# chsl/PLADE

Hardware: AMD Instinct MI355X
Metric: scan-pair registrations/sec, 1M-pt synthetic pairs (higher is better)
Workload: dtype f32

## Files before the change

### include/plade_hip.h

```cpp
#ifndef PLADE_HIP_H
#define PLADE_HIP_H
#include <stddef.h>
#include <stdint.h>
#ifdef __cplusplus
extern "C" {
#endif

#define PLADE_OK 0
#define PLADE_EINVAL (-1)
#define PLADE_EDEVICE (-2)
#define PLADE_ECAP (-3)
#define PLADE_EFAIL (-4)
#define PLADE_ELIMIT (-5)

#define PLADE_GROUP_MAX 8

typedef struct plade_ctx plade_ctx;
typedef struct plade_cloud plade_cloud;
typedef struct plade_comm plade_comm;

int plade_ctx_create(int device, plade_ctx **out);
void plade_ctx_destroy(plade_ctx *ctx);
const char *plade_last_error(const plade_ctx *ctx);
const char *plade_version(void);
// ... 382 lines not shown

int plade_dump_get(plade_ctx *ctx, const char *name, const void **ptr, int64_t *nbytes);
int plade_stats_get(plade_ctx *ctx, const char **names, const double **values, int32_t *count);
int plade_sort_pairs(plade_ctx *ctx, const void *keys, const uint32_t *vals, uint32_t n, int key_bytes, int bits,
                     void *keys_out, uint32_t *vals_out);
int plade_sort_segments(plade_ctx *ctx, const uint32_t *keys, const uint32_t *vals, const uint32_t *seg_off, uint32_t nseg, int bits,
                        uint32_t *keys_out, uint32_t *vals_out);

int plade_selftest_readback(plade_ctx *ctx, uint32_t n_ranges, uint32_t words, uint32_t *mismatches);

int plade_diag_launches(plade_ctx *ctx, uint32_t count, uint32_t blocks, uint32_t mbytes);
int plade_ply_read(const char *path, float **pos_nrm, uint64_t *n, char *err, size_t err_cap);
int plade_ply_read_points(const char *path, float **pos_nrm, uint64_t *n, int32_t *has_normals, char *err, size_t err_cap);
void plade_ply_free(float *pos_nrm);
int plade_diag_cluster_order(const float *sizes, uint32_t n, int32_t mode, int32_t depth_limit, int32_t *order);
int plade_diag_line_solver_host(int32_t kind, const float *a, const float *b, const float *c, const float *d, uint32_t n,
                                float *o1, float *o2, int32_t *ok);
int plade_kernel_time(plade_ctx *ctx, const char *which, int iters, double *avg_seconds,
                      double *algorithmic_bytes_per_launch);

#ifdef __cplusplus
}
#endif
#endif
```

### plade_amd/__init__.py

```python
import ctypes as C
import os
import numpy as np

_HERE = os.path.dirname(os.path.abspath(__file__))
LIB_PATH = os.path.join(_HERE, "libplade_hip.so")

PLADE_OK = 0
PLADE_EINVAL, PLADE_EDEVICE, PLADE_ECAP, PLADE_EFAIL, PLADE_ELIMIT = -1, -2, -3, -4, -5

ABI_SYMBOLS = [
    "plade_ctx_create", "plade_ctx_destroy", "plade_last_error", "plade_version", "plade_default_params",
    "plade_set_params", "plade_score_planes", "plade_extract_planes", "plade_match_descriptors",
    "plade_overlap_counts", "plade_average_spacing", "plade_voxel_downsample", "plade_registration_planes",
    "plade_registration", "plade_registration_minsupport", "plade_cloud_upload", "plade_cloud_free",
    "plade_registration_dev", "plade_dump_get", "plade_stats_get", "plade_kernel_time", "plade_plane_component",
    "plade_sort_pairs", "plade_host_pin", "plade_host_unpin", "plade_score_planes_subset", "plade_registration_next", "plade_cluster_transforms", "plade_device_synchronize", "plade_selftest_readback",
    "plade_registration_pairs", "plade_registration_pairs_dev", "plade_pair_ctx", "plade_set_candidate_shard", "plade_diag_launches", "plade_diag_cluster_order", "plade_diag_line_solver_host", "plade_sort_segments",
    "plade_closest_points", "plade_lines_meet", "plade_ply_read", "plade_ply_free",
    "plade_device_count", "plade_comm_unique_id", "plade_comm_create", "plade_comm_all_gather", "plade_comm_destroy", "plade_comm_last_error",
    "plade_set_candidate_shard_comm",
    "plade_estimate_normals", "plade_cloud_upload_xyz", "plade_ply_read_points",
    "plade_icp_default_params", "plade_refine_icp", "plade_refine_icp_dev", "plade_icp_linearize",
    "plade_cloud_distances", "plade_cloud_distances_dev",
    "plade_outlier_default_params", "plade_filter_outliers", "plade_cloud_filter_outliers_dev",
    "plade_merge_clouds", "plade_merge_clouds_dev", "plade_cloud_download",
    "plade_component_default_params", "plade_label_components", "plade_cloud_filter_components_dev",
    "plade_smooth_default_params", "plade_smooth_cloud", "plade_cloud_smooth_dev",
    "plade_gicp_default_params", "plade_refine_gicp", "plade_refine_gicp_dev", "plade_gicp_linearize",
    "plade_m3c2_default_params", "plade_cloud_m3c2", "plade_cloud_m3c2_dev",
    "plade_fpfh_default_params", "plade_cloud_fpfh", "plade_cloud_fpfh_dev", "plade_features_free",
    "plade_feature_match_default_params", "plade_match_features", "plade_match_features_dev",
    "plade_corr_pose_default_params", "plade_estimate_pose_corr", "plade_estimate_pose_corr_dev", "plade_corr_pose_moments",
# ... 176 lines not shown
    sig("plade_penetration_filter", argtypes=[p, p, u32, p, p, p, p, p, u32, p, p, p, p, p, u32, f, f, p, p, u64, p])
    sig("plade_overlap_counts", argtypes=[p, p, u32, p, u32, p, u32, p, f, f, p])
    sig("plade_average_spacing", argtypes=[p, p, u32, u32, u32, u32, p])
    sig("plade_voxel_downsample", argtypes=[p, p, u32, u32, f, p, p])
    sig("plade_registration_planes", argtypes=[p, p, u32, p, u32, p, p, p, u32, p, p, p, u32, p])
    sig("plade_registration", argtypes=[p, p, u32, p, u32, p])
    sig("plade_registration_next", argtypes=[p, p, u32, p, u32, p, u32, p, u32, p])
    sig("plade_registration_pairs", argtypes=[p, u32, p, p, p, p, u32, p, p, p, p, p, p])
    sig("plade_registration_pairs_dev", argtypes=[p, u32, p, p, p, p])
    sig("plade_pair_ctx", argtypes=[p, u32], restype=p)
    sig("plade_closest_points", argtypes=[p, i32, p, p, p, p, u32, p, p, p, p])
    sig("plade_lines_meet", argtypes=[p, i32, p, p, p, p, u32, p, p])
    sig("plade_diag_launches", argtypes=[p, u32, u32, u32])
    sig("plade_diag_cluster_order", argtypes=[p, u32, i32, i32, p])
    sig("plade_diag_line_solver_host", argtypes=[i32, p, p, p, p, u32, p, p, p])
    sig("plade_ply_read", argtypes=[C.c_char_p, C.POINTER(C.POINTER(C.c_float)), C.POINTER(u64), C.c_char_p, C.c_size_t])
    sig("plade_ply_free", argtypes=[C.POINTER(C.c_float)], restype=None)
    sig("plade_ply_read_points", argtypes=[C.c_char_p, C.POINTER(C.POINTER(C.c_float)), C.POINTER(u64), C.POINTER(i32), C.c_char_p,
                                           C.c_size_t])
    sig("plade_estimate_normals", argtypes=[p, p, u32, u32, i32, p, p, p, p])
    sig("plade_cloud_upload_xyz", argtypes=[p, p, u32, u32, i32, p, C.POINTER(p)])
    sig("plade_icp_default_params", argtypes=[C.POINTER(IcpParams)], restype=None)
    sig("plade_refine_icp", argtypes=[p, p, u32, p, u32, p, C.POINTER(IcpParams), p, C.POINTER(IcpResult)])
    sig("plade_refine_icp_dev", argtypes=[p, p, p, p, C.POINTER(IcpParams), p, C.POINTER(IcpResult)])
    sig("plade_icp_linearize", argtypes=[p, p, u32, p, u32, u32, p, p, f, p, p])
    sig("plade_gicp_default_params", argtypes=[C.POINTER(GicpParams)], restype=None)
    sig("plade_refine_gicp", argtypes=[p, p, u32, p, u32, p, C.POINTER(GicpParams), p, C.POINTER(GicpResult)])
    sig("plade_refine_gicp_dev", argtypes=[p, p, p, p, C.POINTER(GicpParams), p, C.POINTER(GicpResult)])
    sig("plade_gicp_linearize", argtypes=[p, p, u32, p, u32, p, p, f, C.c_double, p, p])
    sig("plade_cloud_distances", argtypes=[p, p, u32, p, u32, u32, p, f, p, p, p, C.POINTER(DistanceSummary)])
# ... 381 lines not shown
    if rc != 0:
        raise PladeError(rc, "plade_diag_line_solver_host failed")
    return (o1, o2, ok) if kind == 0 else (o1, ok)


def cluster_order(sizes, mode=0, depth_limit=-1):
    a = _f32(sizes).reshape(-1)
    out = np.zeros(len(a), np.int32)
    rc = load_library().plade_diag_cluster_order(a.ctypes.data_as(C.c_void_p), len(a), int(mode), int(depth_limit),
                                                 out.ctypes.data_as(C.c_void_p))
    if rc != 0:
        raise PladeError(rc, "plade_diag_cluster_order failed")
    return out


class Cloud:

    def __init__(self, ctx, pos_nrm, handle=None):
        self.ctx = ctx
        if handle is not None:
            self.n, self.h = handle
            return
        a = _f32(pos_nrm)
        if a.ndim != 2 or a.shape[1] != 6:
            raise ValueError(f"Cloud: an (N, 6) array x y z nx ny nz is required, got shape {a.shape}")
        self.n = len(a)
        self.h = C.c_void_p()
        ctx._check(ctx.L.plade_cloud_upload(ctx.h, _ptr(a), self.n, C.byref(self.h)))

    def download(self):
# ... 845 lines not shown
```

### plade_amd/csrc/combiner.hip

```cpp
#include "ctx.h"
#include <algorithm>

namespace plade {

namespace {
constexpr int RANGES_MAX = 32;
struct RangeArgs { const uint32_t *src[RANGES_MAX]; uint32_t *dst[RANGES_MAX]; uint32_t words[RANGES_MAX], value[RANGES_MAX], n; };

template <bool FILL>
__global__ __launch_bounds__(256) void k_ranges(const RangeArgs a, uint32_t *__restrict__ counter, uint32_t *flag, uint32_t seq) {
    const uint32_t r = blockIdx.y, n = a.words[r];
    uint32_t *__restrict__ dst = a.dst[r];
    if (FILL) {
        const uint32_t v = a.value[r];
        for (uint32_t i = blockIdx.x * 256u + threadIdx.x; i < n; i += gridDim.x * 256u) dst[i] = v;
    } else {
        const uint32_t *__restrict__ src = a.src[r];
        for (uint32_t i = blockIdx.x * 256u + threadIdx.x; i < n; i += gridDim.x * 256u) dst[i] = src[i];
    }
    if (!flag) return;
    __threadfence_system();
    __syncthreads();
    if (threadIdx.x == 0) {
        const uint32_t t = atomicAdd(counter, 1u);
// ... 28 lines not shown
    c->comb = this;
    c->comb_slot = slot;
    q[slot].clear();
    ++members;
    return slot;
}

QEntry &Combiner::push(plade_ctx *c) {
    std::vector<QEntry> &v = q[c->comb_slot];
    v.emplace_back();
    ++asked[c->comb_slot];
    return v.back();
}

static bool trace_lockstep() { static const bool v = getenv("PLADE_TRACE_LOCKSTEP") != nullptr; return v; }

void Combiner::flush_locked(std::unique_lock<std::mutex> &lk) {
    (void)lk;
    ++waits;
    const bool tr = trace_lockstep();
    const Clock::time_point t_in = Clock::now();
    size_t n_q = 0;
    uint64_t issued0 = launches_issued;
    if (tr) for (int s = 0; s < BATCH_MAX; ++s) n_q += q[s].size();
    Clock::time_point t_issued = t_in;
    struct TraceOut {
        Combiner *c; bool on; const Clock::time_point &t_in, &t_issued; size_t &n_q; uint64_t &issued0;
        ~TraceOut() {
            if (!on) return;
            const Clock::time_point t_out = Clock::now();
// ... 23 lines not shown
                if (n > best_n) { best_n = n; best = s; }
            }
            if (best < 0) break;
            const QEntry &lead_e = q[best][cur[best]];
            QEntry *es[BATCH_MAX];
            int n = 0;
            if (lead_e.kind == QEntry::FUNC) { es[n++] = &q[best][cur[best]]; ++cur[best]; }
            else
                for (int t = 0; t < BATCH_MAX; ++t) {
                    if (cur[t] >= q[t].size()) continue;
                    QEntry &f = q[t][cur[t]];
                    if (f.kind == lead_e.kind && f.id == lead_e.id) { es[n++] = &f; ++cur[t]; }
                }
            switch (es[0]->kind) {
                case QEntry::KERNEL:
                    es[0]->launch_many(st, n, es);
                    HIP_TRY(hipGetLastError());
                    ++launches_issued;
                    break;
                case QEntry::FUNC:
                    es[0]->fn(st);
                    HIP_TRY(hipGetLastError());
                    ++launches_issued;
                    break;
                case QEntry::COPY_IN:
                case QEntry::FILL: {
                    RangeArgs a;
                    memset(&a, 0, sizeof(a));
                    const QEntry::Kind kind = es[0]->kind;
                    auto put = [&](const QEntry &e) {
// ... 125 lines not shown
    c->read_arena_used = 0; c->write_arena_used = 0;
    c->comb = nullptr;
    c->comb_slot = -1;
}

void Combiner::bury(std::vector<void *> &gy) {
    std::lock_guard<std::mutex> lk(m);
    graveyard.insert(graveyard.end(), gy.begin(), gy.end());
    gy.clear();
}
Combiner::~Combiner() {
    for (void *p : graveyard) dev_free(p);
}

}
```

### plade_amd/csrc/k_overlap.hip

```cpp
#include "overlap.h"
#include "prims.h"

namespace plade {

struct GridParams {
    float mnx, mny, mnz, inv;
    int dx, dy, dz;
};

__device__ void k_minmax3(const VB &vb, const float *__restrict__ xyz, uint32_t n, uint32_t stride, float *__restrict__ out6) {
    __shared__ float s_lds[6][8];
    float mn[3] = {INFINITY, INFINITY, INFINITY}, mx[3] = {-INFINITY, -INFINITY, -INFINITY};
    for (uint32_t i = vb.bx * blockDim.x + threadIdx.x; i < n; i += vb.gx * blockDim.x)
        for (int k = 0; k < 3; ++k) {
            float v = xyz[(size_t)i * stride + k];
            mn[k] = fminf(mn[k], v);
            mx[k] = fmaxf(mx[k], v);
        }
    block_minmax_commit<3>(mn, mx, reinterpret_cast<int *>(out6), s_lds);
}

__device__ __forceinline__ uint32_t block_of(int cx, int cy, int cz, int dx, int dy) {
    const int bdx = (dx + 3) >> 2, bdy = (dy + 3) >> 2;
    return (uint32_t)((cx >> 2) + bdx * ((cy >> 2) + bdy * (cz >> 2)));
// ... 218 lines not shown
        return;
    }
    cell_start.ensure(ncells); cell_end.ensure(ncells);
    ctx->fill_async(cell_start.p, 0, ncells * 4);
    ctx->fill_async(cell_end.p, 0, ncells * 4);
    launch<k_gather_cells, 256>(ctx, dim3(cdiv(n, 256)), 0, d_xyz, stride, keys2.p, vals2.p, n,
                       sorted.p, cell_start.p, cell_end.p);
    HIP_TRY(hipGetLastError());
}

constexpr int OV_TPB = 256;
#ifndef OVD_W
#define OVD_W 5
#endif
constexpr int OV_KCH = 16;
constexpr uint32_t OV_MASK_MAX = 48u << 10;

__device__ void k_overlap(const VB &vb, const float *__restrict__ sx, const float *__restrict__ sy,
                                                    const float *__restrict__ sz, uint32_t n_s,
                                                    const float4 *__restrict__ tgt,
                                                    const unsigned long long *__restrict__ occ_bits,
                                                    const uint32_t *__restrict__ occ_rank,
                                                    const uint32_t *__restrict__ occ_start,
                                                    const float4 *__restrict__ cell_first,
                                                    const uint32_t *__restrict__ blk_mask, uint32_t mask_words, GridParams g,
                                                    const float *__restrict__ T ,
                                                    const float *__restrict__ centers , uint32_t K, float R2,
                                                    float r2, int32_t *__restrict__ counts, uint32_t ch, uint32_t items_per_wg) {
    __shared__ float s_T[OV_KCH][12];
    __shared__ float s_c[OV_KCH][3];
    __shared__ uint32_t s_cnt[OV_KCH];
    extern __shared__ uint32_t s_mask[];
    for (uint32_t i = threadIdx.x; i < mask_words; i += OV_TPB) s_mask[i] = blk_mask[i];
    const int lane = threadIdx.x & 63;
    const uint32_t ntiles = (n_s + OV_TPB - 1) / OV_TPB, nchunks = (K + ch - 1) / ch;
    const uint64_t nitems = (uint64_t)ntiles * nchunks;
    const uint64_t it0 = (uint64_t)vb.bx * items_per_wg, it1 = min(nitems, it0 + items_per_wg);
    uint32_t cur = 0xffffffffu, k0 = 0, kc = 0;
    for (uint64_t item = it0; item < it1; ++item) {
        const uint32_t chunk = (uint32_t)(item / ntiles), tile = (uint32_t)(item % ntiles);
        if (chunk != cur) {
            __syncthreads();
            if (cur != 0xffffffffu && threadIdx.x < kc && s_cnt[threadIdx.x]) atomicAdd(&counts[k0 + threadIdx.x], (int32_t)s_cnt[threadIdx.x]);
            __syncthreads();
            cur = chunk; k0 = chunk * ch; kc = min(ch, K - k0);
            for (uint32_t i = threadIdx.x; i < kc * 12; i += OV_TPB) s_T[i / 12][i % 12] = T[(size_t)(k0 + i / 12) * 16 + i % 12];
            for (uint32_t i = threadIdx.x; i < kc * 3; i += OV_TPB) s_c[i / 3][i % 3] = centers[(size_t)(k0 + i / 3) * 3 + i % 3];
            if (threadIdx.x < OV_KCH) s_cnt[threadIdx.x] = 0u;
            __syncthreads();
        }
        const uint32_t i = tile * OV_TPB + threadIdx.x;
        const bool live = i < n_s;
        const f3 p = live ? f3(sx[i], sy[i], sz[i]) : f3();
// ... 77 lines not shown
                }
            }
            const uint32_t h = (uint32_t)__popcll(__ballot(hit));
            if (lane == 0 && h) atomicAdd(&s_cnt[kk], h);
        }
    }
    __syncthreads();
    if (cur != 0xffffffffu && threadIdx.x < kc && s_cnt[threadIdx.x]) atomicAdd(&counts[k0 + threadIdx.x], (int32_t)s_cnt[threadIdx.x]);
}

__device__ void k_overlap_dense(const VB &vb, const float *__restrict__ sx, const float *__restrict__ sy, const float *__restrict__ sz,
                                uint32_t n_s, const float4 *__restrict__ tgt, const uint32_t *__restrict__ row_start,
                                const uint32_t *__restrict__ near_mask, uint32_t mask_words, int ms,
                                const uint32_t *__restrict__ row_occ , GridParams g,
                                const float *__restrict__ T , const float *__restrict__ centers , uint32_t K, float R2,
                                float r2, int32_t *__restrict__ counts, uint32_t ch, uint32_t items_per_wg) {
    __shared__ float s_T[OV_KCH][12];
    __shared__ float s_c[OV_KCH][3];
    __shared__ uint32_t s_cnt[OV_KCH];
    extern __shared__ uint32_t s_mask[];
    for (uint32_t i = threadIdx.x; i < mask_words; i += OV_TPB) s_mask[i] = near_mask[i];
    const int lane = threadIdx.x & 63;
    const uint32_t ntiles = (n_s + OV_TPB - 1) / OV_TPB, nchunks = (K + ch - 1) / ch;
    const uint64_t nitems = (uint64_t)ntiles * nchunks;
    const uint64_t it0 = (uint64_t)vb.bx * items_per_wg, it1 = min(nitems, it0 + items_per_wg);
    const uint32_t DX = (uint32_t)g.dx + 4u, DY = (uint32_t)g.dy + 4u;
    const uint32_t MBX = ((DX - 1u) >> ms) + 1u, MBY = ((DY - 1u) >> ms) + 1u;
    const uint32_t RS = DX, SS = DX * DY;
    const float fdx = (float)(g.dx + 1), fdy = (float)(g.dy + 1), fdz = (float)(g.dz + 1);
    uint32_t cur = 0xffffffffu, k0 = 0, kc = 0;
    for (uint64_t item = it0; item < it1; ++item) {
        const uint32_t chunk = (uint32_t)(item / ntiles), tile = (uint32_t)(item % ntiles);
        if (chunk != cur) {
            __syncthreads();
            if (cur != 0xffffffffu && threadIdx.x < kc && s_cnt[threadIdx.x]) atomicAdd(&counts[k0 + threadIdx.x], (int32_t)s_cnt[threadIdx.x]);
            __syncthreads();
            cur = chunk; k0 = chunk * ch; kc = min(ch, K - k0);
            for (uint32_t i = threadIdx.x; i < kc * 12; i += OV_TPB) s_T[i / 12][i % 12] = T[(size_t)(k0 + i / 12) * 16 + i % 12];
            for (uint32_t i = threadIdx.x; i < kc * 3; i += OV_TPB) s_c[i / 3][i % 3] = centers[(size_t)(k0 + i / 3) * 3 + i % 3];
            if (threadIdx.x < OV_KCH) s_cnt[threadIdx.x] = 0u;
            __syncthreads();
        }
        const uint32_t i = tile * OV_TPB + threadIdx.x;
        const bool live = i < n_s;
        const f3 p = live ? f3(sx[i], sy[i], sz[i]) : f3();
// ... 124 lines not shown
    if (!n_s) return;
    work.bbox.ensure(8);
    launch<k_init_minmax6, 64>(ctx, dim3(1), 0, work.bbox.p);
    launch<k_src_minmax, 256>(ctx, dim3(std::min(cdiv(n_s, 256), 512u)), 0, d_sx, d_sy, d_sz, n_s,
                       work.bbox.p);
    work.keys.ensure(n_s); work.keys2.ensure(n_s); work.vals.ensure(n_s); work.vals2.ensure(n_s);
    work.sorted.ensure(3 * (size_t)n_s + 4);
    launch<k_src_keys, 256>(ctx, dim3(cdiv(n_s, 256)), 0, d_sx, d_sy, d_sz, n_s, work.bbox.p, 1.f / cell,
                       work.keys.p, work.vals.p);
    sort_pairs_u32(ctx, work.keys.p, work.keys2.p, work.vals.p, work.vals2.p, n_s, 24);
    launch<k_src_gather, 256>(ctx, dim3(cdiv(n_s, 256)), 0, d_sx, d_sy, d_sz, n_s, work.vals2.p,
                       work.sorted.p);
    HIP_TRY(hipGetLastError());
}

void overlap_counts(plade_ctx *ctx, OverlapWork &work, const float *d_sx, const float *d_sy, const float *d_sz, uint32_t n_s,
                    const TargetGrid &grid, const float *d_T, const float *d_centers, uint32_t K, float src_radius,
                    float inlier_dist, int32_t *d_counts, uint32_t *d_any, bool counts_are_zero) {
    if (counts_are_zero) {}
    else if (reinterpret_cast<uint32_t *>(d_counts) + K == d_any) ctx->fill_async(d_counts, 0, (size_t)K * 8);
    else {
        ctx->fill_async(d_counts, 0, (size_t)K * 4);
        ctx->fill_async(d_any, 0, (size_t)K * 4);
    }
    if (K == 0 || grid.n == 0) return;
    const float R2 = pcl_r2((double)src_radius), r2 = pcl_r2((double)inlier_dist);
    GridParams g{grid.gp.mnx, grid.gp.mny, grid.gp.mnz, grid.gp.inv, grid.gp.dx, grid.gp.dy, grid.gp.dz};
    for (uint32_t k0 = 0; k0 < K; k0 += 2048) {
        uint32_t kc = std::min(2048u, K - k0);
        launch<k_sphere_any, 256>(ctx, dim3(cdiv(grid.n, 256)), kc * 12, grid.sorted.p, grid.n,
                           d_centers + (size_t)k0 * 3, kc, R2, d_any + k0);
    }
    if (n_s) {
        uint32_t ch = K <= 64 ? 2u : (K <= 512 ? 4u : (uint32_t)OV_KCH);
        if (grid.dense && K > 512) ch = 8u;
        const uint64_t nitems = (uint64_t)cdiv(n_s, OV_TPB) * cdiv(K, ch);
        const uint32_t fill = 256u * OVD_W / (uint32_t)std::max(1, ctx->comb ? ctx->comb->size() : 1);
        const uint32_t wgs = (uint32_t)std::min<uint64_t>(nitems, grid.dense ? std::max(64u, fill) : (ctx->comb ? 512u : 2048u));
        const uint32_t per = (uint32_t)((nitems + wgs - 1) / wgs);
        ctx->ev_begin("overlap", (double)K * n_s * 12.0 + (double)grid.n * 12.0);
        PLADE_REQUIRE(grid.compact, PLADE_EINVAL, "overlap: the target grid needs the compact occupancy index");
        if (grid.dense) {
            launch<k_overlap_dense, OV_TPB, OVD_W>(ctx, dim3(cdiv(nitems, per)), grid.mask_words * 4, d_sx, d_sy, d_sz, n_s, grid.sorted.p,
                               grid.row_start.p, grid.near_mask.p, grid.mask_words, grid.mask_shift,
                               grid.row_occ_on ? (const uint32_t *)grid.row_occ.p : (const uint32_t *)nullptr, g, d_T, d_centers, K, R2, r2, d_counts,
                               ch, per);
            ctx->ev_end();
            HIP_TRY(hipGetLastError());
            return;
        }
        const uint32_t nw = (uint32_t)((grid.ncells + 63) / 64);
        const uint32_t mask_words = (nw + 31) / 32 * 4 <= OV_MASK_MAX ? (nw + 63) / 64 * 2 : 0u;
        launch<k_overlap, OV_TPB, 5>(ctx, dim3(cdiv(nitems, per)), mask_words * 4, d_sx, d_sy, d_sz, n_s, grid.sorted.p,
                           grid.occ_bits.p, grid.occ_rank.p, grid.occ_start.p, grid.cell_first.p, reinterpret_cast<const uint32_t *>(grid.occ_blk.p), mask_words, g,
                           d_T, d_centers, K, R2, r2, d_counts, ch, per);
        ctx->ev_end();
    }
    HIP_TRY(hipGetLastError());
}

__global__ void k_deinterleave3(const float *__restrict__ xyz, uint32_t n, float *__restrict__ x, float *__restrict__ y,
                                float *__restrict__ z) {
    uint32_t i = blockIdx.x * blockDim.x + threadIdx.x;
    if (i >= n) return;
    x[i] = xyz[3 * (size_t)i]; y[i] = xyz[3 * (size_t)i + 1]; z[i] = xyz[3 * (size_t)i + 2];
}

void deinterleave3(plade_ctx *ctx, const float *d_xyz, uint32_t n, float *d_x, float *d_y, float *d_z) {
    if (!n) return;
    launch_raw(ctx, k_deinterleave3, dim3(cdiv(n, 256)), dim3(256), 0, d_xyz, n, d_x, d_y, d_z);
    HIP_TRY(hipGetLastError());
}

}

using namespace plade;

extern "C" int plade_overlap_counts(plade_ctx *ctx, const float *src_ds, uint32_t n_s, const float *tgt_ds,
                                    uint32_t n_t, const float *T, uint32_t k, const float *centers, float src_radius,
                                    float inlier_dist, int32_t *counts) {
    return guarded(ctx, [&]() -> int {
        PLADE_REQUIRE(src_ds && tgt_ds && T && centers && counts, PLADE_EINVAL, "plade_overlap_counts: null argument");
        DBuf<float> d_src, d_tgt, d_soa, d_T, d_c;
        DBuf<int32_t> d_counts;
        DBuf<uint32_t> d_any;
        d_src.ensure((size_t)n_s * 3 + 4); d_tgt.ensure((size_t)n_t * 3 + 4); d_soa.ensure((size_t)n_s * 3 + 4);
        d_T.ensure((size_t)k * 16 + 4); d_c.ensure((size_t)k * 3 + 4); d_counts.ensure(k + 1); d_any.ensure(k + 1);
        ctx->h2d(d_src.p, src_ds, (size_t)n_s * 12);
        ctx->h2d(d_tgt.p, tgt_ds, (size_t)n_t * 12);
        ctx->h2d(d_T.p, T, (size_t)k * 64);
        ctx->h2d(d_c.p, centers, (size_t)k * 12);
        deinterleave3(ctx, d_src.p, n_s, d_soa.p, d_soa.p + n_s, d_soa.p + 2 * (size_t)n_s);
        TargetGrid grid;
        grid.build(ctx, d_tgt.p, n_t, 3, inlier_dist, nullptr, nullptr, true);
        OverlapWork ow;
        if (n_t && n_s) overlap_sort_source(ctx, ow, d_soa.p, d_soa.p + n_s, d_soa.p + 2 * (size_t)n_s, n_s, 1.f / grid.gp.inv);
        else ow.sorted.ensure(3 * (size_t)n_s + 4);
        overlap_counts(ctx, ow, ow.sorted.p, ow.sorted.p + n_s, ow.sorted.p + 2 * (size_t)n_s, n_s, grid, d_T.p, d_c.p, k, src_radius,
                       inlier_dist, d_counts.p, d_any.p);
        std::vector<uint32_t> any(k);
        ctx->d2h(counts, d_counts.p, (size_t)k * 4);
        ctx->d2h(any.data(), d_any.p, (size_t)k * 4);
        ctx->sync();
        for (uint32_t i = 0; i < k; ++i)
            if (!any[i]) counts[i] = -1;
        return PLADE_OK;
    });
}
```

### plade_amd/csrc/launch.h

```cpp
#pragma once
#include "common.h"
#include <condition_variable>
#include <functional>
#include <mutex>
#include <type_traits>

struct plade_ctx;

namespace plade {

struct VB { uint32_t bx, by, gx, gy; };

constexpr int BATCH_MAX = 8;
constexpr size_t PACK_MAX = 464;

template <class... A> struct Pack;
template <> struct Pack<> {};
template <class H, class... T> struct Pack<H, T...> { H head; Pack<T...> tail; };

template <class... A> inline Pack<A...> make_pack(A... a);
template <> inline Pack<> make_pack<>() { return Pack<>{}; }
template <class H, class... T> inline Pack<H, T...> make_pack_impl(H h, T... t) { Pack<H, T...> p; p.head = h; p.tail = make_pack<T...>(t...); return p; }
template <class... A> inline Pack<A...> make_pack(A... a) { return make_pack_impl<A...>(a...); }

// ... 14 lines not shown

template <auto Body, int TPB, int N, class P, int MINW = 1>
__global__ __launch_bounds__(TPB, MINW) void k_batch(const BatchHdr h, const BatchPacks<P, N> packs) {
    uint32_t e = 0;
    if (N > 1) {
#pragma unroll
        for (int q = 1; q < N; ++q) e += (q < (int)h.n && blockIdx.x >= h.start[q]) ? 1u : 0u;
    }
    const uint32_t lin = blockIdx.x - h.start[e], gx = h.gx[e];
    VB vb;
    vb.bx = lin % gx; vb.by = lin / gx; vb.gx = gx; vb.gy = h.gy[e];
    call_body<Body>(vb, packs.p[e]);
}
#endif

struct QEntry {
    enum Kind : uint8_t { KERNEL, COPY_IN, FILL, FUNC } kind = KERNEL;
    const void *id = nullptr;
    void (*launch_many)(hipStream_t, int, QEntry *const *) = nullptr;
    uint32_t gx = 0, gy = 0, smem = 0;
    void *dst = nullptr; const void *src = nullptr; uint32_t words = 0, value = 0;
    std::function<void(hipStream_t)> fn;
    alignas(16) unsigned char pack[PACK_MAX];
};

struct Combiner {
    plade_ctx *lead = nullptr;
    std::mutex m;
    std::condition_variable cv;
    int members = 0, arrived = 0;
    uint64_t epoch = 0;
    std::string error;
    int error_code = 0;
    plade_ctx *member[BATCH_MAX] = {};
    std::vector<QEntry> q[BATCH_MAX];
// ... 31 lines not shown
        h.n = (uint32_t)k;
        for (int q = 0; q < k; ++q) {
            const QEntry &e = *es[b + q];
            h.gx[q] = std::max(1u, e.gx); h.gy[q] = std::max(1u, e.gy);
            h.start[q + 1] = h.start[q] + e.gx * e.gy;
            memcpy(static_cast<void *>(&packs.p[q]), e.pack, sizeof(P));
            smem = std::max(smem, e.smem);
        }
        for (int q = k; q < BATCH_MAX; ++q) h.start[q + 1] = h.start[k];
        if (h.start[k] == 0) continue;
        hipLaunchKernelGGL((k_batch<Body, TPB, N, P, MINW>), dim3(h.start[k]), dim3(TPB), smem, st, h, packs);
    }
}

template <auto Body, int TPB, int MINW = 1, class... Args>
void launch(plade_ctx *ctx, dim3 grid, size_t smem, Args... args) {
    using Tr = BodyTraits<decltype(Body)>;
    using P = typename Tr::pack;
    static_assert(std::is_trivially_copyable<P>::value, "kernel arguments must be plain data");
    const P p = Tr::make(args...);
    if (grid.x == 0 || grid.y == 0) return;
    Combiner *cb = ctx_combiner(ctx);
    if (!cb || sizeof(P) > PACK_MAX) {
        if (cb) {
            QEntry &e = cb->push(ctx);
            e.kind = QEntry::FUNC;
            e.fn = [p, grid, smem](hipStream_t st) {
                BatchHdr h; memset(&h, 0, sizeof(h));
                h.n = 1; h.gx[0] = grid.x; h.gy[0] = grid.y;
                for (int q = 0; q < BATCH_MAX; ++q) h.start[q + 1] = grid.x * grid.y;
                BatchPacks<P, 1> packs; packs.p[0] = p;
// ... 1 lines not shown
            };
            return;
        }
        BatchHdr h; memset(&h, 0, sizeof(h));
        h.n = 1; h.gx[0] = grid.x; h.gy[0] = grid.y;
        for (int q = 0; q < BATCH_MAX; ++q) h.start[q + 1] = grid.x * grid.y;
        BatchPacks<P, 1> packs; packs.p[0] = p;
        hipLaunchKernelGGL((k_batch<Body, TPB, 1, P, MINW>), dim3(grid.x * grid.y), dim3(TPB), smem, ctx_stream(ctx), h, packs);
        return;
    }
    QEntry &e = cb->push(ctx);
    e.kind = QEntry::KERNEL;
    e.launch_many = &launch_many_impl<Body, TPB, P, MINW>;
    e.id = reinterpret_cast<const void *>(e.launch_many);
    e.gx = grid.x; e.gy = grid.y; e.smem = (uint32_t)smem;
    memcpy(e.pack, static_cast<const void *>(&p), sizeof(P));
}
#endif

}
```

### plade_amd/csrc/overlap.h

```cpp
#pragma once
#include "ctx.h"

namespace plade {

struct TargetGrid {
    struct { float mnx, mny, mnz, inv; int dx, dy, dz; } gp;
    uint32_t n = 0;
    size_t ncells = 0;
    DBuf<float> bbox;
    DBuf<uint32_t> keys, keys2, vals, vals2, cell_start, cell_end;
    DBuf<float4> sorted;
    DBuf<unsigned long long> occ_bits;
    DBuf<unsigned long long> occ_blk;
    DBuf<uint32_t> occ_pop, occ_rank;
    DBuf<uint32_t> occ_start;
    DBuf<float4> cell_first;
    bool compact = false;
    bool dense = false;
    int DX = 0, DY = 0, DZ = 0, mask_shift = 2;
    uint32_t mask_words = 0;
    DBuf<uint32_t> row_start, near_mask;
    DBuf<uint32_t> row_occ;
    bool row_occ_on = false;
    void build(plade_ctx *ctx, const float *d_xyz, uint32_t n_pts, uint32_t stride, float min_cell,
               const float *bbox_min = nullptr, const float *bbox_max = nullptr,
               bool compact_index = false);
};

struct OverlapWork {
    DBuf<uint32_t> keys, keys2, vals, vals2;
    DBuf<float> sorted;
    DBuf<int> bbox;
};
void overlap_sort_source(plade_ctx *ctx, OverlapWork &work, const float *d_sx, const float *d_sy, const float *d_sz, uint32_t n_s,
                         float cell);
void overlap_counts(plade_ctx *ctx, OverlapWork &work, const float *d_sx, const float *d_sy, const float *d_sz, uint32_t n_s,
                    const TargetGrid &grid, const float *d_T, const float *d_centers, uint32_t K, float src_radius,
                    float inlier_dist, int32_t *d_counts, uint32_t *d_any, bool counts_are_zero = false);

void deinterleave3(plade_ctx *ctx, const float *d_xyz, uint32_t n, float *d_x, float *d_y, float *d_z);

}
```

### plade_amd/csrc/pipeline.hip

```cpp
#include "pipeline.h"
#include "hostgeom.h"
#include "prims.h"
#include "exact_sort.h"
#include <algorithm>
#include <numeric>
#include <thread>

namespace plade {

namespace {

struct LengthIndex { float length; int index; };
inline bool cmp_greater(const LengthIndex &a, const LengthIndex &b) { return a.length > b.length; }

__device__ void k_gather_rt(const VB &vb, const float4 *__restrict__ rt, const uint32_t *__restrict__ ids, uint32_t n,
                            float *__restrict__ out ) {
    const uint32_t i = vb.bx * blockDim.x + threadIdx.x;
    if (i >= n) return;
    const uint32_t k = ids[i];
    const float4 r0 = rt[4 * (size_t)k], r1 = rt[4 * (size_t)k + 1], r2 = rt[4 * (size_t)k + 2];
    float *o = out + 12 * (size_t)i;
    o[0] = r0.x; o[1] = r0.y; o[2] = r0.z; o[3] = r1.x; o[4] = r1.y; o[5] = r1.z; o[6] = r2.x; o[7] = r2.y; o[8] = r2.z;
    o[9] = r0.w; o[10] = r1.w; o[11] = r2.w;
}
// ... 409 lines not shown
        T[3] = r[9]; T[7] = r[10]; T[11] = r[11];
        T[12] = T[13] = T[14] = 0.f; T[15] = 1.f;
        const f3 cc = mul_e(R, C.bcenter) + f3(r[9], r[10], r[11]);
        centers[3 * i] = cc.x; centers[3 * i + 1] = cc.y; centers[3 * i + 2] = cc.z;
    }
    std::vector<int32_t> counts(Kv);
    {
        StageTimer t(ctx, "t_verify");
        const plade_ctx::CandidateShard &sh = ctx->shard;
        const bool sharded = ((sh.world > 1 && sh.exchange) || sh.comm) && Kv >= sh.min_candidates;
        const bool by_rccl = sharded && sh.comm;
        std::vector<uint32_t> mine;
        for (uint32_t i = 0; i < Kv; ++i) if (!sharded || i % sh.world == sh.rank) mine.push_back(i);
        const uint32_t Km = (uint32_t)mine.size();
        const uint32_t per = by_rccl ? cdiv(Kv, sh.world) : Km;
        W.d_T16.ensure(19 * (size_t)Km + 2 * (size_t)per + 4);
        float *d_centers = W.d_T16.p + 16 * (size_t)Km;
        int32_t *d_counts = reinterpret_cast<int32_t *>(W.d_T16.p + 19 * (size_t)Km);
        uint32_t *d_any = reinterpret_cast<uint32_t *>(d_counts) + per;
        std::vector<float> up(19 * (size_t)Km + 2 * (size_t)per, 0.f);
        for (uint32_t q = 0; q < Km; ++q) {
            memcpy(up.data() + 16 * (size_t)q, T16.data() + 16 * (size_t)mine[q], 64);
            memcpy(up.data() + 16 * (size_t)Km + 3 * (size_t)q, centers.data() + 3 * (size_t)mine[q], 12);
        }
        std::vector<int32_t> back(2 * (size_t)Kv, 0);
        if (Km || by_rccl) {
            ctx->h2d(W.d_T16.p, up.data(), 4 * up.size());
            if (Km) {
                if (!ctx->comb) HIP_TRY(hipStreamWaitEvent(ctx->stream, W.ev_grid, 0));
                const float *vsx = sort_source ? W.ov_work.sorted.p : C.d_ds_soa.p;
                overlap_counts(ctx, W.ov_work, vsx, vsx + C.n_ds, vsx + 2 * (size_t)C.n_ds, C.n_ds,
                               W.grid, W.d_T16.p, d_centers, Km, (float)C.radius, downSampleDistance, d_counts, d_any, true);
            }
            if (by_rccl) {
                int32_t *d_all = W.d_shard_all.ensure(2 * (size_t)per * sh.world + 4);
                {
                    plade_comm *comm = sh.comm;
                    const size_t bytes = 8 * (size_t)per;
                    ctx->raw_launch([comm, d_counts, d_all, bytes](hipStream_t st) { comm_all_gather_dev(comm, d_counts, d_all, bytes, st); });
                }
                std::vector<int32_t> all(2 * (size_t)per * sh.world);
                ctx->d2h(all.data(), d_all, 4 * all.size());
                ctx->sync();
                for (uint32_t r = 0; r < sh.world; ++r)
                    for (uint32_t q = 0; q < per; ++q) {
                        const uint32_t i = q * sh.world + r;
                        if (i < Kv) { back[i] = all[2 * (size_t)per * r + q]; back[Kv + i] = all[2 * (size_t)per * r + per + q]; }
// ... 82 lines not shown
```

Measured before the change: 797.6.

## Use atomic work-stealing tickets and weighted grid split in overlap kernels

Replaces the static per-workgroup item ranges in the overlap kernels with dynamic claiming through an atomic ticket counter, handing out small chunks of items so workgroups balance load. Adds an elastic grid mechanism in the combiner that splits a shared workgroup budget across batched dense overlap launches in proportion to their work, rather than giving each an equal share. The ticket word rides in the already-uploaded counts buffer so it is zeroed without an extra fill. The aim is to cut tail imbalance and underfilled GPU time when several registrations are combined, at the cost of one atomic and barrier per claim.

```diff
diff --git a/include/plade_hip.h b/include/plade_hip.h
--- a/include/plade_hip.h
+++ b/include/plade_hip.h
@@ -420,6 +420,7 @@
 int plade_ply_read_points(const char *path, float **pos_nrm, uint64_t *n, int32_t *has_normals, char *err, size_t err_cap);
 void plade_ply_free(float *pos_nrm);
 int plade_diag_cluster_order(const float *sizes, uint32_t n, int32_t mode, int32_t depth_limit, int32_t *order);
+int plade_diag_elastic_split(const uint64_t *weights, uint32_t n, uint32_t target, uint32_t *gx);
 int plade_diag_line_solver_host(int32_t kind, const float *a, const float *b, const float *c, const float *d, uint32_t n,
                                 float *o1, float *o2, int32_t *ok);
 int plade_kernel_time(plade_ctx *ctx, const char *which, int iters, double *avg_seconds,
diff --git a/plade_amd/__init__.py b/plade_amd/__init__.py
--- a/plade_amd/__init__.py
+++ b/plade_amd/__init__.py
@@ -15,7 +15,7 @@
     "plade_registration", "plade_registration_minsupport", "plade_cloud_upload", "plade_cloud_free",
     "plade_registration_dev", "plade_dump_get", "plade_stats_get", "plade_kernel_time", "plade_plane_component",
     "plade_sort_pairs", "plade_host_pin", "plade_host_unpin", "plade_score_planes_subset", "plade_registration_next", "plade_cluster_transforms", "plade_device_synchronize", "plade_selftest_readback",
-    "plade_registration_pairs", "plade_registration_pairs_dev", "plade_pair_ctx", "plade_set_candidate_shard", "plade_diag_launches", "plade_diag_cluster_order", "plade_diag_line_solver_host", "plade_sort_segments",
+    "plade_registration_pairs", "plade_registration_pairs_dev", "plade_pair_ctx", "plade_set_candidate_shard", "plade_diag_launches", "plade_diag_cluster_order", "plade_diag_line_solver_host", "plade_diag_elastic_split", "plade_sort_segments",
     "plade_closest_points", "plade_lines_meet", "plade_ply_read", "plade_ply_free",
     "plade_device_count", "plade_comm_unique_id", "plade_comm_create", "plade_comm_all_gather", "plade_comm_destroy", "plade_comm_last_error",
     "plade_set_candidate_shard_comm",
@@ -222,6 +222,7 @@
     sig("plade_diag_launches", argtypes=[p, u32, u32, u32])
     sig("plade_diag_cluster_order", argtypes=[p, u32, i32, i32, p])
     sig("plade_diag_line_solver_host", argtypes=[i32, p, p, p, p, u32, p, p, p])
+    sig("plade_diag_elastic_split", argtypes=[p, u32, u32, p])
     sig("plade_ply_read", argtypes=[C.c_char_p, C.POINTER(C.POINTER(C.c_float)), C.POINTER(u64), C.c_char_p, C.c_size_t])
     sig("plade_ply_free", argtypes=[C.POINTER(C.c_float)], restype=None)
     sig("plade_ply_read_points", argtypes=[C.c_char_p, C.POINTER(C.POINTER(C.c_float)), C.POINTER(u64), C.POINTER(i32), C.c_char_p,
@@ -633,6 +634,15 @@
     return out
 
 
+def elastic_split(weights, target):
+    w = np.ascontiguousarray(weights, np.uint64).reshape(-1)
+    out = np.zeros(len(w), np.uint32)
+    rc = load_library().plade_diag_elastic_split(w.ctypes.data_as(C.c_void_p), len(w), int(target), out.ctypes.data_as(C.c_void_p))
+    if rc != 0:
+        raise PladeError(rc, "plade_diag_elastic_split failed")
+    return out
+
+
 class Cloud:
 
     def __init__(self, ctx, pos_nrm, handle=None):
diff --git a/plade_amd/csrc/combiner.hip b/plade_amd/csrc/combiner.hip
--- a/plade_amd/csrc/combiner.hip
+++ b/plade_amd/csrc/combiner.hip
@@ -66,6 +66,17 @@
 }
 
 static bool trace_lockstep() { static const bool v = getenv("PLADE_TRACE_LOCKSTEP") != nullptr; return v; }
+
+static void share_elastic_grids(int n, QEntry *const *es) {
+    uint64_t w[BATCH_MAX];
+    uint32_t gx[BATCH_MAX];
+    for (int k = 0; k < n; ++k) {
+        if (!es[k]->elastic.weight || es[k]->elastic.target != es[0]->elastic.target || es[k]->gy != 1) return;
+        w[k] = es[k]->elastic.weight;
+    }
+    if (!elastic_split(w, n, es[0]->elastic.target, gx)) return;
+    for (int k = 0; k < n; ++k) es[k]->gx = gx[k];
+}
 
 void Combiner::flush_locked(std::unique_lock<std::mutex> &lk) {
     (void)lk;
@@ -119,6 +130,7 @@
                 }
             switch (es[0]->kind) {
                 case QEntry::KERNEL:
+                    share_elastic_grids(n, es);
                     es[0]->launch_many(st, n, es);
                     HIP_TRY(hipGetLastError());
                     ++launches_issued;
@@ -274,3 +286,8 @@
 }
 
 }
+
+extern "C" int plade_diag_elastic_split(const uint64_t *weights, uint32_t n, uint32_t target, uint32_t *gx) {
+    if (!weights || !gx || n == 0 || n > 4096) return PLADE_EINVAL;
+    return plade::elastic_split(weights, (int)n, target, gx) ? PLADE_OK : PLADE_EINVAL;
+}
diff --git a/plade_amd/csrc/k_overlap.hip b/plade_amd/csrc/k_overlap.hip
--- a/plade_amd/csrc/k_overlap.hip
+++ b/plade_amd/csrc/k_overlap.hip
@@ -256,7 +256,25 @@
 #define OVD_W 5
 #endif
 constexpr int OV_KCH = 16;
+constexpr long OV_CLAIM = 8;
 constexpr uint32_t OV_MASK_MAX = 48u << 10;
+
+__device__ __forceinline__ bool next_items(const VB &vb, uint64_t nitems, uint32_t *__restrict__ ticket, uint32_t claim, uint32_t *s_tk,
+                                           uint32_t &round, uint64_t &it0, uint64_t &it1) {
+    if (!ticket) {
+        if (round++) return false;
+        it0 = nitems * vb.bx / vb.gx;
+        it1 = nitems * ((uint64_t)vb.bx + 1u) / vb.gx;
+        return it0 < it1;
+    }
+    uint32_t *slot = s_tk + (round++ & 1u);
+    if (threadIdx.x == 0) *slot = atomicAdd(ticket, 1u);
+    __syncthreads();
+    const uint32_t t = (uint32_t)__builtin_amdgcn_readfirstlane((int)*slot);
+    it0 = (uint64_t)t * claim;
+    it1 = min(nitems, it0 + claim);
+    return it0 < nitems;
+}
 
 __device__ void k_overlap(const VB &vb, const float *__restrict__ sx, const float *__restrict__ sy,
                                                     const float *__restrict__ sz, uint32_t n_s,
@@ -268,17 +286,18 @@
                                                     const uint32_t *__restrict__ blk_mask, uint32_t mask_words, GridParams g,
                                                     const float *__restrict__ T ,
                                                     const float *__restrict__ centers , uint32_t K, float R2,
-                                                    float r2, int32_t *__restrict__ counts, uint32_t ch, uint32_t items_per_wg) {
+                                                    float r2, int32_t *__restrict__ counts, uint32_t ch, uint32_t *__restrict__ ticket , uint32_t claim) {
     __shared__ float s_T[OV_KCH][12];
     __shared__ float s_c[OV_KCH][3];
-    __shared__ uint32_t s_cnt[OV_KCH];
+    __shared__ uint32_t s_cnt[OV_KCH], s_tk[2];
     extern __shared__ uint32_t s_mask[];
     for (uint32_t i = threadIdx.x; i < mask_words; i += OV_TPB) s_mask[i] = blk_mask[i];
     const int lane = threadIdx.x & 63;
     const uint32_t ntiles = (n_s + OV_TPB - 1) / OV_TPB, nchunks = (K + ch - 1) / ch;
     const uint64_t nitems = (uint64_t)ntiles * nchunks;
-    const uint64_t it0 = (uint64_t)vb.bx * items_per_wg, it1 = min(nitems, it0 + items_per_wg);
-    uint32_t cur = 0xffffffffu, k0 = 0, kc = 0;
+    uint32_t cur = 0xffffffffu, k0 = 0, kc = 0, round = 0;
+    uint64_t it0, it1;
+    while (next_items(vb, nitems, ticket, claim, s_tk, round, it0, it1))
     for (uint64_t item = it0; item < it1; ++item) {
         const uint32_t chunk = (uint32_t)(item / ntiles), tile = (uint32_t)(item % ntiles);
         if (chunk != cur) {
@@ -386,21 +405,22 @@
                                 const uint32_t *__restrict__ near_mask, uint32_t mask_words, int ms,
                                 const uint32_t *__restrict__ row_occ , GridParams g,
                                 const float *__restrict__ T , const float *__restrict__ centers , uint32_t K, float R2,
-                                float r2, int32_t *__restrict__ counts, uint32_t ch, uint32_t items_per_wg) {
+                                float r2, int32_t *__restrict__ counts, uint32_t ch, uint32_t *__restrict__ ticket , uint32_t claim) {
     __shared__ float s_T[OV_KCH][12];
     __shared__ float s_c[OV_KCH][3];
-    __shared__ uint32_t s_cnt[OV_KCH];
+    __shared__ uint32_t s_cnt[OV_KCH], s_tk[2];
     extern __shared__ uint32_t s_mask[];
     for (uint32_t i = threadIdx.x; i < mask_words; i += OV_TPB) s_mask[i] = near_mask[i];
     const int lane = threadIdx.x & 63;
     const uint32_t ntiles = (n_s + OV_TPB - 1) / OV_TPB, nchunks = (K + ch - 1) / ch;
     const uint64_t nitems = (uint64_t)ntiles * nchunks;
-    const uint64_t it0 = (uint64_t)vb.bx * items_per_wg, it1 = min(nitems, it0 + items_per_wg);
     const uint32_t DX = (uint32_t)g.dx + 4u, DY = (uint32_t)g.dy + 4u;
     const uint32_t MBX = ((DX - 1u) >> ms) + 1u, MBY = ((DY - 1u) >> ms) + 1u;
     const uint32_t RS = DX, SS = DX * DY;
     const float fdx = (float)(g.dx + 1), fdy = (float)(g.dy + 1), fdz = (float)(g.dz + 1);
-    uint32_t cur = 0xffffffffu, k0 = 0, kc = 0;
+    uint32_t cur = 0xffffffffu, k0 = 0, kc = 0, round = 0;
+    uint64_t it0, it1;
+    while (next_items(vb, nitems, ticket, claim, s_tk, round, it0, it1))
     for (uint64_t item = it0; item < it1; ++item) {
         const uint32_t chunk = (uint32_t)(item / ntiles), tile = (uint32_t)(item % ntiles);
         if (chunk != cur) {
@@ -555,15 +575,25 @@
     HIP_TRY(hipGetLastError());
 }
 
+static long env_number(const char *name, long none) {
+    const char *v = getenv(name);
+    if (!v || !*v) return none;
+    char *end = nullptr;
+    const long x = strtol(v, &end, 10);
+    return end && *end == 0 && x >= 0 ? x : none;
+}
+
 void overlap_counts(plade_ctx *ctx, OverlapWork &work, const float *d_sx, const float *d_sy, const float *d_sz, uint32_t n_s,
                     const TargetGrid &grid, const float *d_T, const float *d_centers, uint32_t K, float src_radius,
-                    float inlier_dist, int32_t *d_counts, uint32_t *d_any, bool counts_are_zero) {
+                    float inlier_dist, int32_t *d_counts, uint32_t *d_any, bool counts_are_zero, uint32_t *d_ticket) {
+    const bool one_block = reinterpret_cast<uint32_t *>(d_counts) + K == d_any;
     if (counts_are_zero) {}
-    else if (reinterpret_cast<uint32_t *>(d_counts) + K == d_any) ctx->fill_async(d_counts, 0, (size_t)K * 8);
+    else if (one_block) ctx->fill_async(d_counts, 0, ((size_t)K * 2 + (d_ticket == d_any + K ? 1 : 0)) * 4);
     else {
         ctx->fill_async(d_counts, 0, (size_t)K * 4);
         ctx->fill_async(d_any, 0, (size_t)K * 4);
     }
+    if (!counts_are_zero && d_ticket && !(one_block && d_ticket == d_any + K)) ctx->fill_async(d_ticket, 0, 4);
     if (K == 0 || grid.n == 0) return;
     const float R2 = pcl_r2((double)src_radius), r2 = pcl_r2((double)inlier_dist);
     GridParams g{grid.gp.mnx, grid.gp.mny, grid.gp.mnz, grid.gp.inv, grid.gp.dx, grid.gp.dy, grid.gp.dz};
@@ -576,25 +606,31 @@
         uint32_t ch = K <= 64 ? 2u : (K <= 512 ? 4u : (uint32_t)OV_KCH);
         if (grid.dense && K > 512) ch = 8u;
         const uint64_t nitems = (uint64_t)cdiv(n_s, OV_TPB) * cdiv(K, ch);
-        const uint32_t fill = 256u * OVD_W / (uint32_t)std::max(1, ctx->comb ? ctx->comb->size() : 1);
-        const uint32_t wgs = (uint32_t)std::min<uint64_t>(nitems, grid.dense ? std::max(64u, fill) : (ctx->comb ? 512u : 2048u));
-        const uint32_t per = (uint32_t)((nitems + wgs - 1) / wgs);
+        const uint32_t target = 256u * OVD_W;
+        const uint32_t fill = target / (uint32_t)std::max(1, ctx->comb ? ctx->comb->size() : 1);
+        uint32_t wgs = (uint32_t)std::min<uint64_t>(nitems, grid.dense ? std::max(64u, fill) : (ctx->comb ? 512u : 2048u));
+        ElasticGrid el;
+        if (grid.dense && ctx->comb && env_number("PLADE_OVERLAP_EQUAL_SHARES", 0) == 0) { el.weight = nitems; el.target = target; }
+        const long forced = ctx->comb ? -1 : env_number("PLADE_OVERLAP_WGS", -1);
+        if (forced > 0) wgs = (uint32_t)std::min<long>(forced, 1l << 20);
+        uint32_t claim = (uint32_t)std::min<long>(env_number("PLADE_OVERLAP_CLAIM", OV_CLAIM), 1l << 20);
+        if (!d_ticket || !claim || (nitems + claim - 1) / claim + (1ull << 21) >= (1ull << 32)) { d_ticket = nullptr; claim = 0; }
         ctx->ev_begin("overlap", (double)K * n_s * 12.0 + (double)grid.n * 12.0);
         PLADE_REQUIRE(grid.compact, PLADE_EINVAL, "overlap: the target grid needs the compact occupancy index");
         if (grid.dense) {
-            launch<k_overlap_dense, OV_TPB, OVD_W>(ctx, dim3(cdiv(nitems, per)), grid.mask_words * 4, d_sx, d_sy, d_sz, n_s, grid.sorted.p,
+            launch_elastic<k_overlap_dense, OV_TPB, OVD_W>(ctx, el, dim3(wgs), grid.mask_words * 4, d_sx, d_sy, d_sz, n_s, grid.sorted.p,
                                grid.row_start.p, grid.near_mask.p, grid.mask_words, grid.mask_shift,
                                grid.row_occ_on ? (const uint32_t *)grid.row_occ.p : (const uint32_t *)nullptr, g, d_T, d_centers, K, R2, r2, d_counts,
-                               ch, per);
+                               ch, d_ticket, claim);
             ctx->ev_end();
             HIP_TRY(hipGetLastError());
             return;
         }
         const uint32_t nw = (uint32_t)((grid.ncells + 63) / 64);
         const uint32_t mask_words = (nw + 31) / 32 * 4 <= OV_MASK_MAX ? (nw + 63) / 64 * 2 : 0u;
-        launch<k_overlap, OV_TPB, 5>(ctx, dim3(cdiv(nitems, per)), mask_words * 4, d_sx, d_sy, d_sz, n_s, grid.sorted.p,
+        launch<k_overlap, OV_TPB, 5>(ctx, dim3(wgs), mask_words * 4, d_sx, d_sy, d_sz, n_s, grid.sorted.p,
                            grid.occ_bits.p, grid.occ_rank.p, grid.occ_start.p, grid.cell_first.p, reinterpret_cast<const uint32_t *>(grid.occ_blk.p), mask_words, g,
-                           d_T, d_centers, K, R2, r2, d_counts, ch, per);
+                           d_T, d_centers, K, R2, r2, d_counts, ch, d_ticket, claim);
         ctx->ev_end();
     }
     HIP_TRY(hipGetLastError());
@@ -624,9 +660,9 @@
         PLADE_REQUIRE(src_ds && tgt_ds && T && centers && counts, PLADE_EINVAL, "plade_overlap_counts: null argument");
         DBuf<float> d_src, d_tgt, d_soa, d_T, d_c;
         DBuf<int32_t> d_counts;
-        DBuf<uint32_t> d_any;
         d_src.ensure((size_t)n_s * 3 + 4); d_tgt.ensure((size_t)n_t * 3 + 4); d_soa.ensure((size_t)n_s * 3 + 4);
-        d_T.ensure((size_t)k * 16 + 4); d_c.ensure((size_t)k * 3 + 4); d_counts.ensure(k + 1); d_any.ensure(k + 1);
+        d_T.ensure((size_t)k * 16 + 4); d_c.ensure((size_t)k * 3 + 4); d_counts.ensure(2 * (size_t)k + 4);
+        uint32_t *d_any = reinterpret_cast<uint32_t *>(d_counts.p) + k;
         ctx->h2d(d_src.p, src_ds, (size_t)n_s * 12);
         ctx->h2d(d_tgt.p, tgt_ds, (size_t)n_t * 12);
         ctx->h2d(d_T.p, T, (size_t)k * 64);
@@ -638,10 +674,10 @@
         if (n_t && n_s) overlap_sort_source(ctx, ow, d_soa.p, d_soa.p + n_s, d_soa.p + 2 * (size_t)n_s, n_s, 1.f / grid.gp.inv);
         else ow.sorted.ensure(3 * (size_t)n_s + 4);
         overlap_counts(ctx, ow, ow.sorted.p, ow.sorted.p + n_s, ow.sorted.p + 2 * (size_t)n_s, n_s, grid, d_T.p, d_c.p, k, src_radius,
-                       inlier_dist, d_counts.p, d_any.p);
+                       inlier_dist, d_counts.p, d_any, false, d_any + k);
         std::vector<uint32_t> any(k);
         ctx->d2h(counts, d_counts.p, (size_t)k * 4);
-        ctx->d2h(any.data(), d_any.p, (size_t)k * 4);
+        ctx->d2h(any.data(), d_any, (size_t)k * 4);
         ctx->sync();
         for (uint32_t i = 0; i < k; ++i)
             if (!any[i]) counts[i] = -1;
diff --git a/plade_amd/csrc/launch.h b/plade_amd/csrc/launch.h
--- a/plade_amd/csrc/launch.h
+++ b/plade_amd/csrc/launch.h
@@ -1,5 +1,6 @@
 #pragma once
 #include "common.h"
+#include <algorithm>
 #include <condition_variable>
 #include <functional>
 #include <mutex>
@@ -52,11 +53,39 @@
 }
 #endif
 
+struct ElasticGrid { uint64_t weight = 0; uint32_t target = 0; };
+inline bool elastic_split(const uint64_t *weight, int n, uint32_t target, uint32_t *gx) {
+    if (n <= 0 || (uint64_t)n > target) return false;
+    typedef unsigned __int128 u128;
+    typedef __int128 i128;
+    u128 W = 0;
+    for (int i = 0; i < n; ++i) { if (!weight[i]) return false; W += weight[i]; }
+    const u128 total = W < (u128)target ? W : (u128)target;
+    uint64_t sum = 0;
+    for (int i = 0; i < n; ++i) {
+        gx[i] = (uint32_t)std::max<uint64_t>(1, (uint64_t)(total * weight[i] / W));
+        sum += gx[i];
+    }
+    while (sum != (uint64_t)total) {
+        const bool add = sum < (uint64_t)total;
+        int best = -1;
+        i128 best_d = 0;
+        for (int i = 0; i < n; ++i) {
+            if (add ? gx[i] >= weight[i] : gx[i] <= 1u) continue;
+            const i128 d = (i128)(total * weight[i]) - (i128)((u128)gx[i] * W);
+            if (best < 0 || (add ? d > best_d : d < best_d)) { best = i; best_d = d; }
+        }
+        if (add) { ++gx[best]; ++sum; } else { --gx[best]; --sum; }
+    }
+    return true;
+}
+
 struct QEntry {
     enum Kind : uint8_t { KERNEL, COPY_IN, FILL, FUNC } kind = KERNEL;
     const void *id = nullptr;
     void (*launch_many)(hipStream_t, int, QEntry *const *) = nullptr;
     uint32_t gx = 0, gy = 0, smem = 0;
+    ElasticGrid elastic;
     void *dst = nullptr; const void *src = nullptr; uint32_t words = 0, value = 0;
     std::function<void(hipStream_t)> fn;
     alignas(16) unsigned char pack[PACK_MAX];
@@ -118,7 +147,7 @@
 }
 
 template <auto Body, int TPB, int MINW = 1, class... Args>
-void launch(plade_ctx *ctx, dim3 grid, size_t smem, Args... args) {
+void launch_elastic(plade_ctx *ctx, ElasticGrid elastic, dim3 grid, size_t smem, Args... args) {
     using Tr = BodyTraits<decltype(Body)>;
     using P = typename Tr::pack;
     static_assert(std::is_trivially_copyable<P>::value, "kernel arguments must be plain data");
@@ -150,8 +179,11 @@
     e.launch_many = &launch_many_impl<Body, TPB, P, MINW>;
     e.id = reinterpret_cast<const void *>(e.launch_many);
     e.gx = grid.x; e.gy = grid.y; e.smem = (uint32_t)smem;
+    if (grid.y == 1) e.elastic = elastic;
     memcpy(e.pack, static_cast<const void *>(&p), sizeof(P));
 }
+template <auto Body, int TPB, int MINW = 1, class... Args>
+void launch(plade_ctx *ctx, dim3 grid, size_t smem, Args... args) { launch_elastic<Body, TPB, MINW>(ctx, ElasticGrid{}, grid, smem, args...); }
 #endif
 
 }
diff --git a/plade_amd/csrc/overlap.h b/plade_amd/csrc/overlap.h
--- a/plade_amd/csrc/overlap.h
+++ b/plade_amd/csrc/overlap.h
@@ -36,7 +36,7 @@
                          float cell);
 void overlap_counts(plade_ctx *ctx, OverlapWork &work, const float *d_sx, const float *d_sy, const float *d_sz, uint32_t n_s,
                     const TargetGrid &grid, const float *d_T, const float *d_centers, uint32_t K, float src_radius,
-                    float inlier_dist, int32_t *d_counts, uint32_t *d_any, bool counts_are_zero = false);
+                    float inlier_dist, int32_t *d_counts, uint32_t *d_any, bool counts_are_zero = false, uint32_t *d_ticket = nullptr);
 
 void deinterleave3(plade_ctx *ctx, const float *d_xyz, uint32_t n, float *d_x, float *d_y, float *d_z);
 
diff --git a/plade_amd/csrc/pipeline.hip b/plade_amd/csrc/pipeline.hip
--- a/plade_amd/csrc/pipeline.hip
+++ b/plade_amd/csrc/pipeline.hip
@@ -447,11 +447,12 @@
         for (uint32_t i = 0; i < Kv; ++i) if (!sharded || i % sh.world == sh.rank) mine.push_back(i);
         const uint32_t Km = (uint32_t)mine.size();
         const uint32_t per = by_rccl ? cdiv(Kv, sh.world) : Km;
-        W.d_T16.ensure(19 * (size_t)Km + 2 * (size_t)per + 4);
+        W.d_T16.ensure(19 * (size_t)Km + 2 * (size_t)per + 1 + 4);
         float *d_centers = W.d_T16.p + 16 * (size_t)Km;
         int32_t *d_counts = reinterpret_cast<int32_t *>(W.d_T16.p + 19 * (size_t)Km);
         uint32_t *d_any = reinterpret_cast<uint32_t *>(d_counts) + per;
-        std::vector<float> up(19 * (size_t)Km + 2 * (size_t)per, 0.f);
+        uint32_t *d_ticket = d_any + per;
+        std::vector<float> up(19 * (size_t)Km + 2 * (size_t)per + 1, 0.f);
         for (uint32_t q = 0; q < Km; ++q) {
             memcpy(up.data() + 16 * (size_t)q, T16.data() + 16 * (size_t)mine[q], 64);
             memcpy(up.data() + 16 * (size_t)Km + 3 * (size_t)q, centers.data() + 3 * (size_t)mine[q], 12);
@@ -463,7 +464,7 @@
                 if (!ctx->comb) HIP_TRY(hipStreamWaitEvent(ctx->stream, W.ev_grid, 0));
                 const float *vsx = sort_source ? W.ov_work.sorted.p : C.d_ds_soa.p;
                 overlap_counts(ctx, W.ov_work, vsx, vsx + C.n_ds, vsx + 2 * (size_t)C.n_ds, C.n_ds,
-                               W.grid, W.d_T16.p, d_centers, Km, (float)C.radius, downSampleDistance, d_counts, d_any, true);
+                               W.grid, W.d_T16.p, d_centers, Km, (float)C.radius, downSampleDistance, d_counts, d_any, true, d_ticket);
             }
             if (by_rccl) {
                 int32_t *d_all = W.d_shard_all.ensure(2 * (size_t)per * sh.world + 4);
```

Measured after the change: 776.2. 0.973x the previous value.
